# schmeing/ReSeq

Hardware: AMD Instinct MI355X
Metric: simulated read-pairs/sec (2x150 bp) (higher is better)
Workload: dtype f64

## Files before the change

reseq_amd/csrc/rsq_host.cpp:

```cpp
#include <stdio.h>
#include "rsq_host.h"
#include "rsq_textio.h"

#include <errno.h>
#include <fcntl.h>
#include <string.h>
#include <sys/mman.h>
#include <sys/stat.h>
#include <unistd.h>
#include <zlib.h>

#include <algorithm>
#include <array>
#include <atomic>
#include <chrono>
#include <exception>
#include <memory>
#include <mutex>

#include <fstream>
#include <thread>

#include "rsq_core.h"

namespace rsq {

Options &options() {
    static Options o;
    return o;
}
namespace {
struct OptionEntry {
    const char *name;
    int64_t Options::*field;
};
const OptionEntry kOptionTable[] = {
    {"fill_mode", &Options::fill_mode},         {"image_tiles", &Options::image_tiles},     {"rate_rows", &Options::rate_rows},
    {"no_indel_skip", &Options::no_indel_skip}, {"force_exact", &Options::force_exact},     {"min_quality_quads", &Options::min_quality_quads},
    {"trace_plan", &Options::trace_plan},       {"trace_prepare", &Options::trace_prepare},
    {"bias_window", &Options::bias_window},     {"window_chunks", &Options::window_chunks}, {"serial_fasta", &Options::serial_fasta},   {"trace_load", &Options::trace_load},
    {"chain_chunk", &Options::chain_chunk},     {"chain_warmup", &Options::chain_warmup},
    {"serial_parse", &Options::serial_parse},   {"parse_stretch", &Options::parse_stretch}, {"mapped_parses", &Options::mapped_parses},
    {"fasta_stretch", &Options::fasta_stretch}, {"overlap", &Options::overlap}, {"specialize", &Options::specialize}, {"job_write_direct", &Options::job_write_direct},             {"job_chunk_bytes", &Options::job_chunk_bytes}, {"host_gzip", &Options::host_gzip}, {"fill_waves", &Options::fill_waves}, {"fasta_no_stage", &Options::fasta_no_stage},
    {"hiprtc_by_name", &Options::hiprtc_by_name}, {"gzip_route", &Options::gzip_route},       {"gzip_stretch", &Options::gzip_stretch},
    {"sieve_lds", &Options::sieve_lds},         {"sieve_lds_bytes", &Options::sieve_lds_bytes}, {"sieve_tracks_mb", &Options::sieve_tracks_mb},
    {"wide_rows", &Options::wide_rows},
};
}
bool set_option(const char *name, int64_t value) {
    for (const OptionEntry &e : kOptionTable)
        if (0 == strcmp(name, e.name)) {
            options().*(e.field) = value;
            return true;
        }
    return false;
}
bool get_option(const char *name, int64_t *value) {
    for (const OptionEntry &e : kOptionTable)
        if (0 == strcmp(name, e.name)) {
            *value = options().*(e.field);
            return true;
        }
    return false;
}
const char *option_names() {
    static const std::string names = [] {
        std::string s;
        for (const OptionEntry &e : kOptionTable) s += (s.empty() ? "" : " ") + std::string(e.name);
        return s;
    }();
    return names.c_str();
}

static size_t pad8(size_t n) { return (8 - (n & 7)) & 7; }

Container::Container(const std::string &path) {
    std::ifstream f(path, std::ios::binary | std::ios::ate);
    if (!f) throw Error("cannot open profile '" + path + "'");
    std::streamsize sz = f.tellg();
    f.seekg(0);
    buf_.resize((size_t)sz);
    if (!f.read(reinterpret_cast<char *>(buf_.data()), sz)) throw Error("cannot read profile '" + path + "'");
    if (buf_.size() < 16 || memcmp(buf_.data(), "RSQPROF1", 8) != 0) throw Error("'" + path + "' is not an RSQP profile container");
    uint32_t version, n;
    memcpy(&version, &buf_[8], 4);
    memcpy(&n, &buf_[12], 4);
    if (version != 1) throw Error("unsupported RSQP version");
    static const size_t kSize[7] = {1, 2, 4, 8, 4, 8, 8};
    size_t pos = 16;
    for (uint32_t i = 0; i < n; ++i) {
        if (pos + 4 > buf_.size()) throw Error("truncated RSQP container");
// ... 1212 lines not shown
```

reseq_amd/csrc/rsq_host.h:

```cpp
#pragma once
#include <stdint.h>

#include <map>
#include <stdexcept>
#include <string>
#include <string.h>
#include <vector>

namespace rsq {

struct Error : std::runtime_error {
    using std::runtime_error::runtime_error;
};

struct Options {
    int64_t fill_mode = -1;
    int64_t image_tiles = 0;
    int64_t rate_rows = 0;
    int64_t no_indel_skip = 0;
    int64_t force_exact = 0;
    int64_t min_quality_quads = 0;
    int64_t trace_plan = 0;
    int64_t trace_prepare = 0;
    int64_t bias_window = 0;
    int64_t window_chunks = 0;
    int64_t trace_load = 0;
    int64_t serial_fasta = 0;
    int64_t fasta_stretch = 0;
    int64_t chain_chunk = 0;
    int64_t chain_warmup = -1;
    int64_t serial_parse = 0;
    int64_t mapped_parses = 0;
    int64_t parse_stretch = 0;
    int64_t job_chunk_bytes = 0;
    int64_t job_write_direct = 0;
    int64_t specialize = 1;
    int64_t fasta_no_stage = 0;
    int64_t fill_waves = 0;
    int64_t host_gzip = 0;
    int64_t gzip_route = -1;
    int64_t gzip_stretch = 0;
    int64_t hiprtc_by_name = 0;
    int64_t sieve_lds = 1;
    int64_t sieve_lds_bytes = 0;
    int64_t sieve_tracks_mb = 4096;
    int64_t wide_rows = 0;
    int64_t overlap = 0;
};
Options &options();
bool set_option(const char *name, int64_t value);
bool get_option(const char *name, int64_t *value);
const char *option_names();

struct Array {
    int dtype = 0;
    std::vector<uint64_t> dims;
    uint64_t count = 0;
    const uint8_t *data = nullptr;
};

class Container {
   public:
    explicit Container(const std::string &path);
    const Array &get(const std::string &name) const;
    bool has(const std::string &name) const { return arrays_.count(name) != 0; }
    template <class T>
    std::vector<T> vec(const std::string &name, int dtype) const {
        const Array &a = get(name);
        if (a.dtype != dtype) throw Error("profile array '" + name + "' has the wrong type");
        const T *p = reinterpret_cast<const T *>(a.data);
        return std::vector<T>(p, p + a.count);
    }
// ... 161 lines not shown
```

reseq_amd/csrc/rsq_pack.h:

```cpp
#pragma once
#include <math.h>
#include <stdio.h>
#include <stdlib.h>
#include <string.h>
#include <errno.h>
#include <fcntl.h>
#include <unistd.h>

#include <algorithm>
#include <string>
#include <vector>

#include <atomic>
#include <exception>
#include <mutex>
#include <thread>

#include "rsq_host.h"
#include "rsq_chains.h"
#include "rsq_sieve.h"
#include "rsq_reads.h"

namespace rsq {

// ... 26 lines not shown

struct SimState {
    Options opt = options();
    Profile prof;
    bool has_ref = false;
    std::vector<std::string> ref_first_names, ref_ids;
    std::vector<uint32_t> seq_len;
    std::vector<uint64_t> seq_word_off, seq_base_off;
    uint64_t total_ref_size = 0;
    uint32_t chain_chunk = 256;
    std::vector<uint64_t> ref_words_host;
    uint32_t ref_code(uint32_t seq, uint32_t pos) const { return (uint32_t)(ref_words_host[seq_word_off[seq] + (pos >> 5)] >> ((pos & 31u) * 2u)) & 3u; }
    bool has_variants = false;
    uint32_t num_alleles = 1;
    int variants_mode = 0;
    std::vector<DevVariant> variants;
    std::vector<uint32_t> var_ptr;
    std::vector<uint8_t> var_bases;
    std::vector<uint16_t> var_err_fwd, var_err_rev;
    uint16_t *dev_var_err_fwd = nullptr, *dev_var_err_rev = nullptr;
    double expected_passing = 0.0;
    std::vector<AlleleVar> allele_map;
    std::vector<uint32_t> allele_map_ptr;
    std::vector<ExtraStart> extra;
    std::vector<uint32_t> extra_seq_ptr;
    std::vector<double> host_pool;
    std::vector<uint8_t> host_par0;
    std::vector<DevTable> host_dom_error, host_error_rate;
    DevSim dev{};
    NameTable names{};
    uint16_t *sys_fwd = nullptr, *sys_rev = nullptr, *adapter_sys[2] = {nullptr, nullptr};
    uint32_t rmax = 0, read_stride = 0, ops_stride = 0, max_adapter = 0, template_words = 0;
    uint64_t insert_lengths_from = 0;
    bool prepared = false;
    uint32_t prepared_lo = 0, prepared_hi = 0;
    uint64_t seed = 0, total_pairs = 0, adapter_only_pairs = 0;
    uint32_t n_groups = 0, passes = 0, total_blocks = 0;
    std::vector<uint32_t> coverage_groups, first_block, n_blocks, block_seq;
    std::vector<double> thresholds, norm_by_len, ref_seq_bias;
    std::string ref_bias_file;
    double bias_normalization = 0;
    std::string plan_note;
    int variants_mode_packed = 0;
    bool has_methylation = false;
    std::vector<uint32_t> meth_ptr_host, meth_first_host, meth_second_host;
    std::vector<double> meth_rate_host;
};

static inline uint32_t cdiv(uint64_t a, uint64_t b) { return (uint32_t)((a + b - 1) / b); }

constexpr uint32_t kLdsBudgetBytes = 160u * 1024u;
constexpr uint32_t kLdsRateRowsFirst = 64;

inline void pack_tables(SimState &s, Uploader &up) {
    const Profile &p = s.prof;
    std::vector<double> pool;
    std::vector<uint8_t> par0;
    auto pack = [&](const std::vector<HostTable> &tabs) {
        std::vector<DevTable> out(tabs.size());
        for (size_t i = 0; i < tabs.size(); ++i) {
            const HostTable &t = tabs[i];
            DevTable d{};
            d.k = (uint32_t)t.par0.size();
            for (uint32_t v : t.par0) d.max_value = std::max(d.max_value, v);
            const uint32_t kp = row_stride(d.k);
            for (uint32_t n = 0; n < t.nm; ++n) {
                d.from[n] = t.from[n];
                d.rows[n] = t.to[n] - t.from[n];
                const size_t rows = d.k ? d.rows[n] : 0;
                if (pool.size() + rows * kp > 0xFFFFFFF0ull) throw Error("probability tables exceed 2^32 entries");
                d.off[n] = (uint32_t)pool.size();
                for (size_t r = 0; r < rows; ++r) {
                    pool.insert(pool.end(), t.dim2[n].begin() + r * d.k, t.dim2[n].begin() + (r + 1) * d.k);
                    pool.insert(pool.end(), kp - d.k, 0.0);
                }
            }
            out[i] = d;
        }
        return out;
    };
    std::vector<DevTable> quality = pack(p.quality), seq_quality = pack(p.seq_quality), base_call = pack(p.base_call), dom_error = pack(p.dom_error),
                          error_rate = pack(p.error_rate), indels = pack(p.indels);

    const uint32_t T = p.n_tiles();
    LdsPlan plan{};
    auto put_par0 = [&](DevTable &d, const HostTable &t) {
        d.par0_off = (uint32_t)par0.size();
        for (uint32_t v : t.par0) par0.push_back((uint8_t)v);
    };
    auto pad_par0 = [&] { par0.resize((par0.size() + 3u) & ~(size_t)3u, 0); };
    for (size_t i = 0; i < indels.size(); ++i) put_par0(indels[i], p.indels[i]);
    pad_par0();
    const uint32_t par0_indel_bytes = (uint32_t)par0.size();
    std::vector<uint32_t> par0_tile_first(2 * T + 1, 0);
    for (uint32_t g = 0; g < 2 * T; ++g) {
        par0_tile_first[g] = (uint32_t)par0.size();
        for (uint32_t i = 0; i < 4; ++i) put_par0(quality[g * 4 + i], p.quality[g * 4 + i]);
        put_par0(seq_quality[g], p.seq_quality[g]);
        for (uint32_t i = 0; i < 20; ++i) put_par0(base_call[g * 20 + i], p.base_call[g * 20 + i]);
        pad_par0();
    }
    par0_tile_first[2 * T] = (uint32_t)par0.size();
    for (size_t i = 0; i < dom_error.size(); ++i) put_par0(dom_error[i], p.dom_error[i]);
    for (size_t i = 0; i < error_rate.size(); ++i) put_par0(error_rate[i], p.error_rate[i]);

    std::vector<float> pool32;
// ... 81 lines not shown
                g.from[n] = any ? std::min(g.from[n], d.from[n]) : d.from[n];
                to[n] = any ? std::max(to[n], d.from[n] + d.rows[n]) : d.from[n] + d.rows[n];
            }
            any = true;
        }
        for (uint32_t n = 0; n < 4; ++n) {
            const uint32_t rows = n < nm ? std::max(1u, to[n] - g.from[n]) : 0u;
            g.before[n] = g.table_rows;
            g.last[n] = rows ? rows - 1u : 0u;
            g.table_rows += rows;
        }
        g.off32 = (uint32_t)pool32.size();
        g.lds = g.lds2 = kNoLds;
        if ((pool32.size() + (uint64_t)tabs.size() * g.table_rows * slot) * sizeof(float) > 0xFFFFFFF0ull)
            throw Error("single-precision probability tables exceed 4 GB (the kernels address them by 32-bit byte offsets)");
        for (DevTable &d : tabs) {
            d.off32 = 0;
            d.f32_ok = 1;
            const uint32_t kp = row_stride(d.k);
            for (uint32_t n = 0; n < nm && d.k; ++n)
                for (uint32_t r = 0; r < d.rows[n]; ++r)
                    for (uint32_t c = 0; c < d.k; ++c) {
                        const double v = pool[d.off[n] + (size_t)r * kp + c];
                        if (!(v == 0.0 || (v >= 0x1p-60 && v <= 0x1p29))) d.f32_ok = 0;
                    }
            const bool zeros = !d.k || !d.f32_ok;
            for (uint32_t n = 0; n < nm; ++n)
                for (uint32_t r = 0; r <= g.last[n]; ++r) {
                    const int64_t own = (int64_t)g.from[n] + r - (int64_t)d.from[n];
                    const double *row = zeros ? nullptr : pool.data() + d.off[n] + (size_t)std::min<int64_t>(std::max<int64_t>(own, 0), (int64_t)d.rows[n] - 1) * kp;
                    for (uint32_t c = 0; c < slot; ++c) pool32.push_back(row && c < d.k ? (float)row[c] : 0.f);
                }
        }
        return g;
    };
    auto family_values = [&](FamilyGeo &g, const std::vector<DevTable> &tabs, uint32_t slot) {
        g.values_src = (uint32_t)par0.size();
        for (const DevTable &d : tabs)
            for (uint32_t c = 0; c < slot; ++c) par0.push_back(c < d.k ? par0[d.par0_off + c] : (uint8_t)0);
    };
    const Options &opt = s.opt;
    const uint32_t min_quads = opt.min_quality_quads > 0 ? (uint32_t)opt.min_quality_quads : 0u;
    for (uint32_t q : kQualityQuads)
        if (!plan.quads_q && q >= min_quads && quads_of(kmax_of(quality)) <= q) plan.quads_q = q;
    const bool screenable = plan.quads_q && quads_of(kmax_of(base_call)) <= kQuadsSmall && quads_of(kmax_of(indels)) <= kQuadsSmall;
    plan.slot_q = row_slot32(plan.quads_q);
    plan.slot_b = plan.slot_i = kSlotSmall;
    if (screenable) {
        plan.q = family(quality, 4, plan.slot_q);
        plan.b = family(base_call, 4, plan.slot_b);
        plan.i = family(indels, 3, plan.slot_i);
        if (!opt.no_indel_skip)
            for (DevTable &d : indels) certain_no_indel(d);
    }
    s.dev.chain_quads = 0;
    s.dev.force_exact = opt.force_exact ? 1u : 0u;
    for (uint32_t q : kChainQuads)
        if (!s.dev.chain_quads && quads_of(kmax_of(error_rate)) <= q && quads_of(kmax_of(dom_error)) <= kQuadsSmall) s.dev.chain_quads = q;
    std::vector<uint32_t> chain_sure(1, 0u);
    if (s.dev.chain_quads) {
        copy32(dom_error, 4u * kQuadsSmall);
        copy32(error_rate, 4u * s.dev.chain_quads);
        if (!opt.no_indel_skip)
            for (DevTable &d : error_rate) {
                d.sure_range = 0;
                if (!d.k || !d.f32_ok || !d.rows[0] || !d.rows[1] || !d.rows[2]) continue;
                uint32_t z = d.k;
                for (uint32_t c = 0; c < d.k; ++c)
                    if (0 == par0[d.par0_off + c]) z = c;
                if (z == d.k) continue;
                const uint32_t kp = row_stride(d.k);
                std::vector<double> worst1(d.k, 0.0);
                for (uint32_t c = 0; c < d.k; ++c)
                    for (uint32_t r = 0; r < d.rows[1] && worst1[c] >= 0.0; ++r) {
                        const double *row = pool.data() + d.off[1] + (size_t)r * kp;
                        if (row[z] > 0.0) worst1[c] = std::max(worst1[c], row[c] / row[z]);
                        else if (row[c] > 0.0) worst1[c] = -1.0;
                    }
                d.sure_range = (uint32_t)chain_sure.size();
                for (uint32_t r0 = 0; r0 < d.rows[0]; ++r0)
                    for (uint32_t r2 = 0; r2 < d.rows[2]; ++r2) {
                        const double *m0 = pool.data() + d.off[0] + (size_t)r0 * kp, *m2 = pool.data() + d.off[2] + (size_t)r2 * kp;
                        double below = 0.0, above = 0.0;
                        bool bound = m0[z] > 0.0 && m2[z] > 0.0;
                        for (uint32_t c = 0; c < d.k && bound; ++c) {
                            if (c == z) continue;
                            if (worst1[c] < 0.0) bound = false;
                            else (c < z ? below : above) += (m0[c] / m0[z]) * worst1[c] * (m2[c] / m2[z]);
                        }
                        uint32_t range = 0;
                        if (bound) {
                            const double lo = above / (1.0 + above) * (1.0 + 1e-9), hi = 1.0 / (1.0 + below) * (1.0 - 1e-9);
                            const uint32_t lo16 = (uint32_t)std::ceil(lo * 65536.0), hi16 = (uint32_t)std::floor(hi * 65536.0);
                            if (lo16 < hi16) range = lo16 | (hi16 << 16);
                        }
                        chain_sure.push_back(range);
                    }
            }
    }
    s.dev.chain_sure = up.put(chain_sure);
    if (screenable) {
        pad_par0();
        family_values(plan.q, quality, plan.slot_q);
        family_values(plan.b, base_call, plan.slot_b);
        family_values(plan.i, indels, plan.slot_i);
    }

    uint32_t rate_rows_q = ~0u, rate_rows_b = ~0u;
    if (opt.rate_rows > 0) rate_rows_q = rate_rows_b = (uint32_t)std::min<int64_t>(opt.rate_rows, 1 << 20);
    rate_rows_q = std::min(rate_rows_q, plan.q.last[3] + 1u);
    rate_rows_b = std::min(rate_rows_b, plan.b.last[3] + 1u);
    const uint64_t budget = kLdsBudgetBytes / 4u - kSchedWords;
    auto plan_image = [&](uint32_t Ti) {
        const uint32_t n_img = 2 * T / Ti;
        uint32_t par0_bytes = 0;
        for (uint32_t g = 0; g < n_img; ++g) par0_bytes = std::max(par0_bytes, par0_indel_bytes + par0_tile_first[(g + 1) * Ti] - par0_tile_first[g * Ti]);
        const uint32_t par0_words = (par0_bytes + 15u) / 16u * 4u;
        const uint32_t desc_words = (lds_desc_count(Ti) * kDescWords + 3u) / 4u * 4u + par0_words;
        const uint32_t values_words = (4 * Ti * plan.slot_q + 20 * Ti * plan.slot_b + 12 * plan.slot_i + 15u) / 16u * 4u;
        const uint32_t rows_q = plan.q.last[0] + 1 + plan.q.last[1] + 1, rows_b = plan.b.last[0] + 1, rows_b2 = plan.b.last[2] + 1, rows_i = plan.i.last[0] + 1;
        auto odd_stride = [](uint64_t floats) { return (uint32_t)(((floats / 4u) | 1u) * 4u); };
        const uint32_t stride_q = odd_stride((uint64_t)rows_q * plan.slot_q), stride_b = odd_stride((uint64_t)rows_b * plan.slot_b), stride_b2 = odd_stride((uint64_t)rows_b2 * plan.slot_b),
                       stride_i = odd_stride((uint64_t)rows_i * plan.slot_i);
        const uint64_t need_q = (uint64_t)4 * Ti * stride_q, need_b = (uint64_t)20 * Ti * stride_b, need_b2 = (uint64_t)20 * Ti * stride_b2, need_i0 = (uint64_t)12 * stride_i;
        uint64_t need = (uint64_t)desc_words + values_words + need_q + need_b;
        auto need_rate = [&](uint32_t rows_q, uint32_t rows_b) {
            return (uint64_t)4 * Ti * odd_stride((uint64_t)rows_q * plan.slot_q) + (uint64_t)20 * Ti * odd_stride((uint64_t)rows_b * plan.slot_b);
        };
        const uint32_t ring_stride = 4 * Ti * plan.slot_q;
        need += (uint64_t)kFillWavesMax * kRingRows * ring_stride;
        if (need + need_rate(1, 1) > budget) return false;
        uint32_t rq = 1, rb = 1;
        while (rq < std::min(rate_rows_q, kLdsRateRowsFirst) && need + need_rate(rq + 1, 1) <= budget) ++rq;
        const bool stage_b2 = need + need_b2 + need_rate(rq, 1) <= budget;
        if (stage_b2) need += need_b2;
        const bool stage_i0 = need + need_i0 + need_rate(rq, 1) <= budget;
        if (stage_i0) need += need_i0;
        while (rb < std::min(rate_rows_b, kLdsRateRowsFirst) && need + need_rate(rq, rb + 1) <= budget) ++rb;
        while (rq < rate_rows_q && need + need_rate(rq + 1, rb) <= budget) ++rq;
        while (rb < rate_rows_b && need + need_rate(rq, rb + 1) <= budget) ++rb;
        plan.img_tiles = Ti;
        plan.binned = (Ti < T || opt.image_tiles == 1) ? 1u : 0u;
        plan.par0_words = par0_words;
        plan.par0_indel_bytes = par0_indel_bytes;
        plan.desc_words = desc_words;
        plan.ring_stride = ring_stride;
        plan.rate_rows_q = rq;
        plan.rate_rows_b = rb;
        plan.q.values = desc_words * 4u;
        plan.b.values = plan.q.values + 4 * Ti * plan.slot_q;
        plan.i.values = plan.b.values + 20 * Ti * plan.slot_b;
        uint32_t at = desc_words + values_words;
        plan.q.lds = at, plan.q.lds_rows = rows_q, plan.q.lds_stride = stride_q, at += (uint32_t)need_q;
        plan.b.lds = at, plan.b.lds_rows = rows_b, plan.b.lds_stride = stride_b, at += (uint32_t)need_b;
        plan.b.lds2 = stage_b2 ? at : kNoLds;
        plan.b.lds2_stride = stride_b2;
        if (stage_b2) at += (uint32_t)need_b2;
        plan.i.lds = stage_i0 ? at : kNoLds;
        plan.i.lds_rows = rows_i;
        plan.i.lds_stride = stride_i;
        if (stage_i0) at += (uint32_t)need_i0;
        plan.ring_off = at;
        plan.q3_off = plan.ring_off + kFillWavesMax * kRingRows * plan.ring_stride;
        plan.q3_stride = odd_stride((uint64_t)plan.rate_rows_q * plan.slot_q);
        plan.b3_stride = odd_stride((uint64_t)plan.rate_rows_b * plan.slot_b);
        plan.b3_off = plan.q3_off + 4 * Ti * plan.q3_stride;
        plan.total_words = plan.b3_off + 20 * Ti * plan.b3_stride;
        plan.mask = plan.quads_q;
        return true;
    };
    plan.img_tiles = T;
    if (screenable && opt.fill_mode != 0) {
        const bool per_tile_first = opt.image_tiles == 1 && T > 1;
        if (!(per_tile_first && plan_image(1)) && !plan_image(T) && !(T > 1 && plan_image(1)))
            s.plan_note = "the read kernels' table image does not fit the " + std::to_string(kLdsBudgetBytes / 1024u) +
                          " KiB of local memory even for one tile: every per-base draw runs in double precision from device memory (several times slower)";
    } else if (!screenable && opt.fill_mode != 0)
        s.plan_note = "the profile's tables are outside what the screened single-precision draws are built for (more than " + std::to_string(4u * kQualityQuads[4]) +
                      " quality values, or more than 8 base-call / indel outcomes): every per-base draw runs in double precision from device memory (several times slower)";
    if ((plan.desc_words | plan.q3_off | plan.b3_off | plan.ring_off | plan.ring_stride | plan.slot_q | plan.slot_b | plan.slot_i | plan.q.off32 | plan.b.off32 | plan.i.off32 |
         (plan.mask ? plan.q.lds | plan.b.lds | (plan.b.lds2 != kNoLds ? plan.b.lds2 : 0u) | (plan.i.lds != kNoLds ? plan.i.lds : 0u) : 0u)) & 3u)
        throw Error("internal: LDS rows must start on 16-byte boundaries");
    if (opt.trace_plan)
        fprintf(stderr, "[rsq] LDS image: mask %u, %u of %u tiles per image, %u words (%u KiB), desc %u, quality slot %u, rate rows %u / %u, q3 %u b3 %u, ring %u x %u, b2 %d i0 %d\n", plan.mask,
                plan.img_tiles, T, plan.total_words, plan.total_words / 256, plan.desc_words, plan.slot_q, plan.rate_rows_q, plan.rate_rows_b, plan.q3_off, plan.b3_off, plan.ring_off,
                plan.ring_stride, (int)(plan.b.lds2 != kNoLds), (int)(plan.i.lds != kNoLds));
    s.dev.lds = plan;
    s.dev.quality = up.put(quality);
    s.dev.seq_quality = up.put(seq_quality);
    s.dev.base_call = up.put(base_call);
    s.dev.dom_error = up.put(dom_error);
    s.dev.error_rate = up.put(error_rate);
    s.dev.indels = up.put(indels);
    par0.resize(((par0.size() + 3u) & ~(size_t)3u) + (size_t)plan.par0_words * 4u + 16u, 0);
    pool.push_back(0.0);
    pool.push_back(0.0);
    pool32.resize(pool32.size() + 8, 0.f);
    s.dev.pool = up.put(pool);
    s.dev.pool32 = up.put(pool32);
    s.dev.par0 = up.put(par0);
    s.host_pool = pool;
    s.host_par0 = par0;
    s.host_dom_error = dom_error;
    s.host_error_rate = error_rate;
}

inline uint32_t effective_fill_mask(uint32_t plan_mask, int forced) { return forced == 0 ? 0u : plan_mask; }

inline void pack_profile(SimState &s, Uploader &up) {
    const Profile &p = s.prof;
    DevSim &d = s.dev;
    d.n_tiles = p.n_tiles();
    d.phred_offset = p.phred_offset;
    d.max_len_deletion = p.max_len_deletion;
    d.reset_distance = p.reset_distance;
    d.tile_cp = up.put(discrete_cp(p.tile_abundance.data(), p.tile_abundance.size()));
    d.tiles = up.put(p.tiles);
    s.rmax = 0;
    uint32_t max_adapter = 0;
    for (int seg = 0; seg < 2; ++seg) {
        const HostAdapters &a = p.adapters[seg];
        DevAdapters &da = d.adapters[seg];
        da.n = a.n();
        da.seqs = up.put(a.seqs);
        da.seq_ptr = up.put(a.seq_ptr);
        da.adapter_cp = up.put(discrete_cp(a.significant.data(), a.significant.size()));
        std::vector<double> cut_cp;
        for (uint32_t i = 0; i < a.n(); ++i) {
            std::vector<double> cp = discrete_cp(a.cut.data() + a.cut_ptr[i], a.cut_ptr[i + 1] - a.cut_ptr[i]);
            cp.resize(a.cut_ptr[i + 1] - a.cut_ptr[i]);
            cut_cp.insert(cut_cp.end(), cp.begin(), cp.end());
            max_adapter = std::max(max_adapter, a.seq_ptr[i + 1] - a.seq_ptr[i]);
        }
        cut_cp.push_back(1.0);
        da.cut_cp = up.put(cut_cp);
        da.cut_ptr = up.put(a.cut_ptr);
        da.cut_from = up.put(a.cut_from);
        s.adapter_sys[seg] = up.put(std::vector<uint16_t>(a.seqs.size() + 1, 0));
        da.sys = s.adapter_sys[seg];
// ... 1259 lines not shown
```

reseq_amd/csrc/rsq_reads.h:

```cpp
#pragma once
#include "rsq_core.h"
#include "rsq_variants.h"
#include "rsq_text.h"

namespace rsq {

struct ReadOut {
    WordColumn seq, qual, ops;
    uint32_t cur_word, cur_index;
    uint32_t seq_word, qual_word, n_put;
    RSQ_HD void put(uint32_t pos, uint32_t base, uint32_t qual_char) {
        const uint32_t sh = (pos & 3u) * 8u;
        seq_word |= base << sh;
        qual_word |= qual_char << sh;
        n_put = pos + 1u;
        if ((pos & 3u) == 3u) {
            seq.at(pos >> 2) = seq_word;
            qual.at(pos >> 2) = qual_word;
            seq_word = qual_word = 0;
        }
    }
    RSQ_HD void op(uint32_t it, uint32_t code) {
        const uint32_t wi = it >> 4;
        if (wi != cur_index) {
// ... 342 lines not shown
    RSQ_HD uint32_t org_len() const { return 0; }
    RSQ_HD uint32_t base(uint32_t) const { return 0; }
    RSQ_HD uint32_t sys_base(uint32_t) const { return 0; }
    RSQ_HD uint32_t sys_deleted(uint32_t) const { return 0; }
};

RSQ_HD uint32_t draw_tile(const DevSim &S, uint32_t c0, uint32_t c1, uint32_t c2, uint32_t c3base) {
    if (RSQ_SIM(S, n_tiles) > 1) return discrete_draw(S.tile_cp, RSQ_SIM(S, n_tiles), u32_to_unit(philox(S.seed, c0, c1, c2, c3base).w0));
    return 0;
}

RSQ_HD uint32_t lds_desc_count(uint32_t n_tiles) { return 25u * n_tiles + 12u; }
RSQ_HD uint32_t image_qbase(const DevSim &S, uint32_t seg, uint32_t first_tile) { return (seg * RSQ_SIM(S, n_tiles) + first_tile) * 4u; }
constexpr uint32_t kDescWords = sizeof(DevTable) / 4u;

#if defined(__HIP_DEVICE_COMPILE__)
#define RSQ_NOINLINE __device__ __noinline__
#else
#define RSQ_NOINLINE inline
#endif
#if defined(RSQ_SCREEN_STATS) && !defined(__HIP_DEVICE_COMPILE__)
#define RSQ_SCREEN_COUNT(family, decided) (++RSQ_SCREEN_STATS[family][0], RSQ_SCREEN_STATS[family][1] += !(decided))
#else
#define RSQ_SCREEN_COUNT(family, decided) ((void)0)
#endif

template <int NM>
#if defined(__HIP_DEVICE_COMPILE__)
__device__ __noinline__
#else
inline
#endif
    uint32_t exact_draw_call(const double *pool, const RSQ_LDS float *img, uint32_t par0_words, uint32_t desc, uint32_t i0, uint32_t i1, uint32_t i2, uint32_t i3, uint32_t word) {
    const DevTable t = reinterpret_cast<const RSQ_LDS DevTable *>(img)[desc];
    uint32_t idx[NM];
    idx[0] = i0;
    idx[1] = i1;
    idx[2] = i2;
    if constexpr (NM == 4) idx[3] = i3;
    double ps;
    const uint32_t value = draw_slim<NM>(t, pool, reinterpret_cast<const RSQ_LDS uint8_t *>(img + par0_words), idx, u32_to_unit(word), ps);
    return value | (0.0 == ps ? 0x80000000u : 0u);
}

#define RSQ_GEO_ROW(S, fam, n, v) ((uint32_t)geo_clamp((int32_t)(v) - (int32_t)RSQ_PLAN(S, fam.from[n]), (int32_t)RSQ_PLAN(S, fam.last[n])))
RSQ_HD int32_t geo_clamp(int32_t d, int32_t last) {
#if defined(__clang__)
    return __builtin_elementwise_min(__builtin_elementwise_max(d, 0), last);
#else
    return d < 0 ? 0 : (d > last ? last : d);
#endif
}

template <uint32_t MASK, int QB = RSQ_SCREEN_BATCH>
struct ScreenTables {
    using Sum = uint32_t;
    static constexpr int QQ = (int)MASK;
    const DevSim &S;
    const RSQ_LDS float *img;
    uint32_t qbase;
    const RSQ_LDS float *ring_;
    uint32_t t;
    uint32_t demand = 0xFFFFFFFFu;
    RSQ_HD DevTable desc(uint32_t local) const { return reinterpret_cast<const RSQ_LDS DevTable *>(img)[local]; }
    RSQ_HD uint32_t par0_at() const { return RSQ_PLAN(S, desc_words) - RSQ_PLAN(S, par0_words); }
    RSQ_HD DevTable quality(uint32_t i) const { return desc(i - qbase); }
    RSQ_HD DevTable seq_quality(uint32_t i) const { return desc(24u * RSQ_PLAN(S, img_tiles) + 12u + i - qbase / 4u); }
    RSQ_HD const RSQ_LDS float *ring(uint32_t p) const { return ring_ + (p % kRingSlots) * RSQ_PLAN(S, ring_stride); }
    RSQ_HD bool in_ring(uint32_t p) const { return t - p <= kRingLag; }
    template <int NM>
    RSQ_HD uint32_t exact(uint32_t desc, const uint32_t (&idx)[NM], uint32_t word, uint32_t &ps) const {
        const uint32_t r = exact_draw_call<NM>(S.pool, img, par0_at(), desc, idx[0], idx[1], idx[2], NM == 4 ? idx[NM - 1] : 0u, word);
        ps = (r >> 31) ^ 1u;
        return r & 0x7FFFFFFFu;
    }
    template <int NM>
    RSQ_HD uint32_t settle(bool decided, uint32_t values, uint32_t column, uint32_t desc, const uint32_t (&idx)[NM], uint32_t u, uint32_t &ps) const {
        uint32_t value = reinterpret_cast<const RSQ_LDS uint8_t *>(img)[values + column];
        ps = 1u;
        decided = decided && !RSQ_SIM(S, force_exact);
        if (!decided) value = exact<NM>(desc, idx, u, ps);
        return value;
    }

    RSQ_HD uint32_t draw_quality(uint32_t i, const uint32_t (&idx)[4], uint32_t u, uint32_t &ps) const {
        const uint32_t local = i - qbase, slot = RSQ_PLAN(S, slot_q), nr = RSQ_PLAN(S, rate_rows_q), r3 = RSQ_GEO_ROW(S, q, 3, idx[3]);
        const RSQ_LDS float *mine = img + RSQ_PLAN(S, q.lds) + local * RSQ_PLAN(S, q.lds_stride);
        const LdsRow32 m0{mine + RSQ_GEO_ROW(S, q, 0, idx[0]) * slot}, m1{mine + (RSQ_PLAN(S, q.before[1]) + RSQ_GEO_ROW(S, q, 1, idx[1])) * slot};
        const bool near = in_ring(idx[2]);
        const LdsRow32 m2{ring_ + (near ? idx[2] % kRingSlots : kRingSlots) * RSQ_PLAN(S, ring_stride) + local * slot};
        const LdsRow32 m3{img + RSQ_PLAN(S, q3_off) + local * RSQ_PLAN(S, q3_stride) + (r3 < nr ? r3 : 0u) * slot};
        uint32_t col = 0;
        const bool decided = draw_screened_batched<QQ, QQ % QB == 0 ? QB : (QQ % 2 == 0 ? 2 : 1)>(u, col, m0, m1, m2, m3) && (near || idx[2] == demand) && r3 < nr;
        RSQ_SCREEN_COUNT(0, decided);
        return settle<4>(decided, RSQ_PLAN(S, q.values), local * slot + col, local, idx, u, ps);
    }
    RSQ_HD uint32_t draw_base_call(uint32_t i, const uint32_t (&idx)[4], uint32_t u, uint32_t &ps) const {
        const uint32_t local = i - qbase * 5u, slot = RSQ_PLAN(S, slot_b), nr = RSQ_PLAN(S, rate_rows_b), r3 = RSQ_GEO_ROW(S, b, 3, idx[3]);
        const uint32_t g = 4u * (RSQ_PLAN(S, b.off32) + i * (RSQ_PLAN(S, b.table_rows) * slot));
        const LdsRow32 m0{img + RSQ_PLAN(S, b.lds) + local * RSQ_PLAN(S, b.lds_stride) + RSQ_GEO_ROW(S, b, 0, idx[0]) * slot};
        const PoolRow32 m1{S.pool32, g + 4u * (RSQ_PLAN(S, b.before[1]) + RSQ_GEO_ROW(S, b, 1, idx[1])) * slot};
        const uint32_t r2 = RSQ_GEO_ROW(S, b, 2, idx[2]);
        const bool m2_staged = RSQ_PLAN(S, b.lds2) != kNoLds, staged = r3 < nr;
        const MixedRow32 m2{LdsRow32{img + (m2_staged ? RSQ_PLAN(S, b.lds2) + local * RSQ_PLAN(S, b.lds2_stride) + r2 * slot : 0u)},
                            PoolRow32{S.pool32, g + 4u * (RSQ_PLAN(S, b.before[2]) + r2) * slot}, m2_staged};
        const MixedRow32 m3{LdsRow32{img + RSQ_PLAN(S, b3_off) + local * RSQ_PLAN(S, b3_stride) + (staged ? r3 : 0u) * slot}, PoolRow32{S.pool32, g + 4u * (RSQ_PLAN(S, b.before[3]) + r3) * slot}, staged};
        uint32_t col = 0;
        const bool decided = draw_screened<(int)kQuadsSmall>(u, col, m0, m1, m2, m3);
        RSQ_SCREEN_COUNT(1, decided);
        return settle<4>(decided, RSQ_PLAN(S, b.values), local * slot + col, 4u * RSQ_PLAN(S, img_tiles) + local, idx, u, ps);
    }
    RSQ_HD uint32_t draw_indel(uint32_t i, const uint32_t (&idx)[3], uint32_t u, uint32_t &ps) const {
        const RSQ_LDS DevTable *d = reinterpret_cast<const RSQ_LDS DevTable *>(img) + (24u * RSQ_PLAN(S, img_tiles) + i);
        const uint32_t range = d->sure_range, lo16 = range & 0xFFFFu;
        const bool sure = (u >> 16) - lo16 < (range >> 16) - lo16 && idx[0] <= d->from[0];
        RSQ_SCREEN_COUNT(3, sure);
        ps = 1u;
        if (sure) return 0;
        const uint32_t slot = RSQ_PLAN(S, slot_i), r0 = RSQ_GEO_ROW(S, i, 0, idx[0]);
        const uint32_t g = 4u * (RSQ_PLAN(S, i.off32) + i * (RSQ_PLAN(S, i.table_rows) * slot));
        const bool m0_staged = RSQ_PLAN(S, i.lds) != kNoLds;
        const MixedRow32 m0{LdsRow32{img + (m0_staged ? RSQ_PLAN(S, i.lds) + i * RSQ_PLAN(S, i.lds_stride) + r0 * slot : 0u)}, PoolRow32{S.pool32, g + 4u * r0 * slot}, m0_staged};
        const PoolRow32 m1{S.pool32, g + 4u * (RSQ_PLAN(S, i.before[1]) + RSQ_GEO_ROW(S, i, 1, idx[1])) * slot}, m2{S.pool32, g + 4u * (RSQ_PLAN(S, i.before[2]) + RSQ_GEO_ROW(S, i, 2, idx[2])) * slot};
        uint32_t col = 0;
        const bool decided = draw_screened<(int)kQuadsSmall>(u, col, m0, m1, m2);
        RSQ_SCREEN_COUNT(2, decided);
        return settle<3>(decided, RSQ_PLAN(S, i.values), i * slot + col, 24u * RSQ_PLAN(S, img_tiles) + i, idx, u, ps);
    }
    RSQ_HD uint32_t draw_seq_quality(uint32_t i, const uint32_t (&idx)[3], uint32_t u, uint32_t &ps) const {
        const uint32_t r = exact_draw_call<3>(S.pool, img, par0_at(), 24u * RSQ_PLAN(S, img_tiles) + 12u + i - qbase / 4u, idx[0], idx[1], idx[2], 0u, u);
        ps = (r >> 31) ^ 1u;
        return r & 0x7FFFFFFFu;
    }
};

RSQ_HD void lds_stage_descriptors(const DevSim &S, RSQ_LDS float *img, uint32_t qbase, uint32_t tid, uint32_t nthreads) {
    const uint32_t T = RSQ_PLAN(S, img_tiles);
    RSQ_LDS uint32_t *dst = reinterpret_cast<RSQ_LDS uint32_t *>(img);
    const uint32_t wq = 4u * T * kDescWords, wb = 20u * T * kDescWords, wi = 12u * kDescWords, ws = T * kDescWords;
    const uint32_t *q = reinterpret_cast<const uint32_t *>(S.quality + qbase), *b = reinterpret_cast<const uint32_t *>(S.base_call + qbase * 5u),
                   *in = reinterpret_cast<const uint32_t *>(S.indels), *sq = reinterpret_cast<const uint32_t *>(S.seq_quality + qbase / 4u);
    const uint32_t tiles_at = S.quality[qbase].par0_off, shift = tiles_at - RSQ_PLAN(S, par0_indel_bytes);
    for (uint32_t i = tid; i < wq; i += nthreads) dst[i] = q[i] - (i % kDescWords == 1u ? shift : 0u);
    for (uint32_t i = tid; i < wb; i += nthreads) dst[wq + i] = b[i] - (i % kDescWords == 1u ? shift : 0u);
    for (uint32_t i = tid; i < wi; i += nthreads) dst[wq + wb + i] = in[i];
    for (uint32_t i = tid; i < ws; i += nthreads) dst[wq + wb + wi + i] = sq[i] - (i % kDescWords == 1u ? shift : 0u);
    const uint32_t *p0 = reinterpret_cast<const uint32_t *>(S.par0), *p1 = reinterpret_cast<const uint32_t *>(S.par0 + tiles_at);
    const uint32_t indel_words = RSQ_PLAN(S, par0_indel_bytes) / 4u, par0_at = RSQ_PLAN(S, desc_words) - RSQ_PLAN(S, par0_words);
    for (uint32_t i = tid; i < RSQ_PLAN(S, par0_words); i += nthreads) dst[par0_at + i] = i < indel_words ? p0[i] : p1[i - indel_words];
    const uint32_t nq = T * RSQ_PLAN(S, slot_q), nb = 5u * T * RSQ_PLAN(S, slot_b), ni = 3u * RSQ_PLAN(S, slot_i);
    const uint32_t *vq = reinterpret_cast<const uint32_t *>(S.par0 + RSQ_PLAN(S, q.values_src)) + qbase / 4u * RSQ_PLAN(S, slot_q),
                   *vb = reinterpret_cast<const uint32_t *>(S.par0 + RSQ_PLAN(S, b.values_src)) + qbase / 4u * 5u * RSQ_PLAN(S, slot_b),
                   *vi = reinterpret_cast<const uint32_t *>(S.par0 + RSQ_PLAN(S, i.values_src));
    for (uint32_t i = tid; i < nq; i += nthreads) dst[RSQ_PLAN(S, q.values) / 4u + i] = vq[i];
    for (uint32_t i = tid; i < nb; i += nthreads) dst[RSQ_PLAN(S, b.values) / 4u + i] = vb[i];
    for (uint32_t i = tid; i < ni; i += nthreads) dst[RSQ_PLAN(S, i.values) / 4u + i] = vi[i];
}
RSQ_HD void lds_stage_family_rows(const DevSim &S, RSQ_LDS float *img, uint32_t off32, uint32_t table_rows, uint32_t first, uint32_t n_tables, uint32_t first_row, uint32_t n_rows,
                                  uint32_t slot, uint32_t dst_off, uint32_t dst_stride, uint32_t tid, uint32_t nthreads) {
    const uint32_t per_table = n_rows * (slot / 4u);
    for (uint32_t i = tid; i < n_tables * per_table; i += nthreads) {
        const uint32_t table = i / per_table, g = i - table * per_table;
        reinterpret_cast<RSQ_LDS Quad *>(img + dst_off + table * dst_stride)[g] = reinterpret_cast<const Quad *>(S.pool32 + off32 + ((size_t)(first + table) * table_rows + first_row) * slot)[g];
    }
}
RSQ_HD void lds_stage_rows(const DevSim &S, RSQ_LDS float *img, uint32_t qbase, uint32_t tid, uint32_t nthreads) {
    const uint32_t T = RSQ_PLAN(S, img_tiles), sq = RSQ_PLAN(S, slot_q), sb = RSQ_PLAN(S, slot_b), si = RSQ_PLAN(S, slot_i);
    lds_stage_family_rows(S, img, RSQ_PLAN(S, q.off32), RSQ_PLAN(S, q.table_rows), qbase, 4u * T, 0u, RSQ_PLAN(S, q.lds_rows), sq, RSQ_PLAN(S, q.lds), RSQ_PLAN(S, q.lds_stride), tid, nthreads);
    lds_stage_family_rows(S, img, RSQ_PLAN(S, b.off32), RSQ_PLAN(S, b.table_rows), qbase * 5u, 20u * T, 0u, RSQ_PLAN(S, b.lds_rows), sb, RSQ_PLAN(S, b.lds), RSQ_PLAN(S, b.lds_stride), tid, nthreads);
    if (RSQ_PLAN(S, b.lds2) != kNoLds)
        lds_stage_family_rows(S, img, RSQ_PLAN(S, b.off32), RSQ_PLAN(S, b.table_rows), qbase * 5u, 20u * T, RSQ_PLAN(S, b.before[2]), RSQ_PLAN(S, b.last[2]) + 1u, sb, RSQ_PLAN(S, b.lds2),
                              RSQ_PLAN(S, b.lds2_stride), tid, nthreads);
    if (RSQ_PLAN(S, i.lds) != kNoLds)
        lds_stage_family_rows(S, img, RSQ_PLAN(S, i.off32), RSQ_PLAN(S, i.table_rows), 0u, 12u, 0u, RSQ_PLAN(S, i.lds_rows), si, RSQ_PLAN(S, i.lds), RSQ_PLAN(S, i.lds_stride), tid, nthreads);
    lds_stage_family_rows(S, img, RSQ_PLAN(S, q.off32), RSQ_PLAN(S, q.table_rows), qbase, 4u * T, RSQ_PLAN(S, q.before[3]), RSQ_PLAN(S, rate_rows_q), sq, RSQ_PLAN(S, q3_off), RSQ_PLAN(S, q3_stride), tid,
                          nthreads);
    lds_stage_family_rows(S, img, RSQ_PLAN(S, b.off32), RSQ_PLAN(S, b.table_rows), qbase * 5u, 20u * T, RSQ_PLAN(S, b.before[3]), RSQ_PLAN(S, rate_rows_b), sb, RSQ_PLAN(S, b3_off), RSQ_PLAN(S, b3_stride), tid,
                          nthreads);
}
RSQ_HD uint32_t lds_ring_items(const DevSim &S) { return 4u * RSQ_PLAN(S, img_tiles) * RSQ_PLAN(S, quads_q); }
struct RingItem {
    uint32_t rows;
    uint32_t at;
};
RSQ_HD RingItem lds_ring_item(const DevSim &S, uint32_t qbase, uint32_t item) {
    const uint32_t table = item / RSQ_PLAN(S, quads_q), c = item % RSQ_PLAN(S, quads_q), slot = RSQ_PLAN(S, slot_q);
    return RingItem{4u * (RSQ_PLAN(S, q.off32) + ((qbase + table) * RSQ_PLAN(S, q.table_rows) + RSQ_PLAN(S, q.before[2])) * slot + 4u * c), table * slot + 4u * c};
}
RSQ_HD Quad lds_ring_load(const DevSim &S, const RingItem &it, uint32_t p) { return PoolRow32{S.pool32, it.rows + 4u * RSQ_GEO_ROW(S, q, 2, p) * RSQ_PLAN(S, slot_q)}.quad(0u); }
RSQ_HD void lds_ring_store(const DevSim &S, const RingItem &it, RSQ_LDS float *ring, uint32_t p, const Quad &q) {
    *reinterpret_cast<RSQ_LDS Quad *>(ring + (p % kRingSlots) * RSQ_PLAN(S, ring_stride) + it.at) = q;
}
RSQ_HD void lds_ring_stage(const DevSim &S, const RingItem &it, RSQ_LDS float *ring, uint32_t p) { lds_ring_store(S, it, ring, p, lds_ring_load(S, it, p)); }
RSQ_HD void lds_ring_stage_demand(const DevSim &S, const RingItem &it, RSQ_LDS float *ring, uint32_t p) {
    *reinterpret_cast<RSQ_LDS Quad *>(ring + kRingSlots * RSQ_PLAN(S, ring_stride) + it.at) = lds_ring_load(S, it, p);
}
RSQ_HD void lds_ring_stage(const DevSim &S, uint32_t qbase, RSQ_LDS float *ring, uint32_t p, uint32_t item) { lds_ring_stage(S, lds_ring_item(S, qbase, item), ring, p); }
RSQ_HD FragmentSrc fragment_src(const DevSim &S, const Fragment &f, uint32_t seg, uint32_t end) {
    const uint32_t L = S.seq_len[f.seq];
    const uint32_t want = S.read_lengths[seg].to + RSQ_SIM(S, max_len_deletion);
    FragmentSrc src;
    src.words = hap_words(S, f.allele);
    src.word_off = S.seq_word_off[f.seq];
    src.len = f.len < want ? f.len : want;
    src.reverse = seg != f.strand;
    src.first = src.reverse ? end : f.start;
    src.sys_ = src.reverse ? S.sys_rev + S.seq_base_off[f.seq] + (L - end) : S.sys_fwd + S.seq_base_off[f.seq] + f.start;
    src.converted = nullptr;
    src.gc_prefix = hap_gc_prefix(S, f.allele);
    return src;
}
RSQ_HD FragmentSrc fragment_src(const DevSim &S, const Fragment &f, uint32_t seg) { return fragment_src(S, f, seg, f.start + f.len); }

struct VariantSrc : FragmentSrc {
    const DevVariant *var;
    const uint16_t *err;
    uint32_t n_var, L, allele;
    uint32_t *walk_error;
    uint32_t spos0, cur0, var_pos0;
    mutable uint32_t spos, cur, var_pos;
    RSQ_HD const DevVariant &var_at(uint32_t i) const { return reverse ? var[n_var - 1u - i] : var[i]; }
    RSQ_HD uint32_t var_spos(uint32_t i) const { return reverse ? L - 1u - var_at(i).pos : var_at(i).pos; }
    RSQ_HD uint32_t var_err(uint32_t i, uint32_t k) const { return err[var_at(i).off + k]; }
    RSQ_HD uint32_t lower_bound(uint32_t sp) const {
        uint32_t lo = 0, hi = n_var;
        while (lo < hi) {
            const uint32_t mid = (lo + hi) >> 1;
            if (var_spos(mid) < sp) lo = mid + 1u;
            else hi = mid;
        }
        return lo;
// ... 592 lines not shown
```

reseq_amd/csrc/rsq_types.h:

```cpp
#pragma once
#if defined(__HIPCC_RTC__)
using __hip_internal::int32_t;
using __hip_internal::int64_t;
using __hip_internal::uint16_t;
using __hip_internal::uint32_t;
using __hip_internal::uint64_t;
using __hip_internal::uint8_t;
typedef unsigned long uintptr_t;
#define RSQ_DEVICE_BUILD 1
#define RSQ_HD __host__ __device__ __forceinline__
#elif defined(__HIPCC__)
#include <stdint.h>
#include <hip/hip_runtime.h>
#define RSQ_DEVICE_BUILD 1
#define RSQ_HD __host__ __device__ __forceinline__
#else
#include <stdint.h>
#define RSQ_DEVICE_BUILD 0
#define RSQ_HD inline
#endif

namespace rsq {

constexpr uint32_t kBlockSize = 1000;
// ... 20 lines not shown
static_assert(__builtin_offsetof(DevTable, par0_off) == 4, "lds_stage_descriptors rewrites word 1 of a descriptor");
constexpr uint32_t kNoLds = 0xFFFFFFFFu;
#ifndef RSQ_CHUNK_LARGE
#define RSQ_CHUNK_LARGE 4
#endif
constexpr uint32_t kChunkSmall = 3, kChunkLarge = RSQ_CHUNK_LARGE;
RSQ_HD uint32_t chunk_pairs(uint32_t k) { return k <= 2u * kChunkSmall ? kChunkSmall : kChunkLarge; }
RSQ_HD uint32_t chunks_of(uint32_t k, uint32_t u) { return (k + 2u * u - 1u) / (2u * u); }
RSQ_HD uint32_t row_stride(uint32_t k) {
    const uint32_t u = chunk_pairs(k), kp = chunks_of(k, u) * 2u * u;
    return (kp & 2u) ? kp : kp + 2u;
}
RSQ_HD uint32_t quads_of(uint32_t k) { return (k + 3u) / 4u; }
RSQ_HD uint32_t row_slot32(uint32_t quads) {
    const uint32_t w = quads * 4u;
    return (w & 4u) ? w : w + 4u;
}
constexpr uint32_t kQuadsSmall = 2, kSlotSmall = 8;
constexpr uint32_t kQualityQuads[] = {3, 6, 10, 11, 12};
constexpr uint32_t kChainQuads[] = {8, 16, 26};
constexpr uint32_t kRingSlots = 2, kRingLag = 1;
constexpr uint32_t kRingRows = kRingSlots + 1u;

struct FamilyGeo {
    uint32_t from[4];
    uint32_t last[4];
    uint32_t before[4];
    uint32_t table_rows;
    uint32_t off32;
    uint32_t lds;
    uint32_t lds_rows;
    uint32_t lds_stride;
    uint32_t lds2;
    uint32_t lds2_stride;
    uint32_t values;
    uint32_t values_src;
};

struct LdsPlan {
    uint32_t mask;
    uint32_t img_tiles;
    uint32_t binned;
    uint32_t desc_words;
    uint32_t par0_words;
    uint32_t par0_indel_bytes;
    uint32_t slot_q, slot_b, slot_i;
    uint32_t quads_q;
    uint32_t rate_rows_q, rate_rows_b;
    uint32_t q3_off, b3_off;
    uint32_t q3_stride, b3_stride;
    uint32_t ring_off, ring_stride;
    uint32_t total_words;
    FamilyGeo q, b, i;
};

struct Fragment {
    uint32_t seq;
    uint32_t start;
    uint32_t len;
    uint16_t dup;
    uint8_t strand;
    uint8_t allele;
    uint32_t block;
    uint32_t number;
};

struct ReadMeta {
    uint16_t read_len;
    uint16_t num_errors;
    uint16_t n_iter_m;
    uint16_t n_iter_s;
    uint16_t hard_clip;
    uint16_t tile_id;
    uint16_t cigar_chars;
    uint16_t plain;
};

struct DevVariant {
    uint32_t pos;
    uint32_t len;
    uint32_t off;
    uint32_t pad;
    uint64_t allele[2];
};
struct AlleleVar {
    uint32_t pos;
    uint32_t vid;
    int32_t shift;
    int32_t gc;
};
struct FragmentVar {
    uint32_t end;
    uint32_t sub;
    int32_t start_var;
    uint32_t start_var_pos;
    int32_t end_var;
    uint32_t end_var_pos;
};
struct ExtraStart {
    uint32_t pos;
    uint32_t sub;
    int32_t first_variant_id;
    uint32_t start_variant_pos;
};

struct DevAdapters {
    uint32_t n;
// ... 105 lines not shown
```

Baseline: 248.3 million.

## Add LDS-staged word screen to skip exact base-call draws

On the host, compute per-table conservative float bounds on the ratio of non-reference to reference base-call probabilities, bucketed over the four conditioning indices. These bounds are packed into pool32 and staged into LDS when the budget allows. In the kernel, the draw first checks whether the uniform word is certain to land on the reference base. If so, it returns that base directly and skips the four-row table lookup and cumulative comparison. The cost is extra LDS space, which can reduce rate rows staged elsewhere, plus a short check on every draw.

```diff
diff --git a/reseq_amd/csrc/rsq_host.cpp b/reseq_amd/csrc/rsq_host.cpp
--- a/reseq_amd/csrc/rsq_host.cpp
+++ b/reseq_amd/csrc/rsq_host.cpp
@@ -36,7 +36,7 @@
 };
 const OptionEntry kOptionTable[] = {
     {"fill_mode", &Options::fill_mode},         {"image_tiles", &Options::image_tiles},     {"rate_rows", &Options::rate_rows},
-    {"no_indel_skip", &Options::no_indel_skip}, {"force_exact", &Options::force_exact},     {"min_quality_quads", &Options::min_quality_quads},
+    {"no_indel_skip", &Options::no_indel_skip}, {"force_exact", &Options::force_exact},     {"base_call_word", &Options::base_call_word},     {"min_quality_quads", &Options::min_quality_quads},
     {"trace_plan", &Options::trace_plan},       {"trace_prepare", &Options::trace_prepare},
     {"bias_window", &Options::bias_window},     {"window_chunks", &Options::window_chunks}, {"serial_fasta", &Options::serial_fasta},   {"trace_load", &Options::trace_load},
     {"chain_chunk", &Options::chain_chunk},     {"chain_warmup", &Options::chain_warmup},
diff --git a/reseq_amd/csrc/rsq_host.h b/reseq_amd/csrc/rsq_host.h
--- a/reseq_amd/csrc/rsq_host.h
+++ b/reseq_amd/csrc/rsq_host.h
@@ -18,6 +18,7 @@
     int64_t image_tiles = 0;
     int64_t rate_rows = 0;
     int64_t no_indel_skip = 0;
+    int64_t base_call_word = 1;
     int64_t force_exact = 0;
     int64_t min_quality_quads = 0;
     int64_t trace_plan = 0;
diff --git a/reseq_amd/csrc/rsq_pack.h b/reseq_amd/csrc/rsq_pack.h
--- a/reseq_amd/csrc/rsq_pack.h
+++ b/reseq_amd/csrc/rsq_pack.h
@@ -102,6 +102,65 @@
 constexpr uint32_t kLdsBudgetBytes = 160u * 1024u;
 constexpr uint32_t kLdsRateRowsFirst = 64;
 
+struct WordScreenGeo {
+    uint32_t at[4], cap[4], stride;
+};
+inline WordScreenGeo word_screen_geo(const FamilyGeo &g) {
+    WordScreenGeo w{};
+    const uint32_t lim[4] = {kWordCapQuality, kWordCapBuckets, kWordCapErrors, kWordCapRate};
+    uint32_t at = 0;
+    for (uint32_t n = 0; n < 4; ++n) {
+        const uint32_t top = (g.from[n] + g.last[n]) >> (1 == n ? kWordPosShift : 0u);
+        w.at[n] = at;
+        w.cap[n] = std::min(top, lim[n]);
+        at += w.cap[n] + 1u;
+    }
+    w.stride = at;
+    return w;
+}
+inline bool base_call_word_bounds(const DevTable &d, const double *pool, const uint8_t *par0, uint32_t base, const FamilyGeo &g, const WordScreenGeo &w, float *out, uint32_t *sides) {
+    const float inf = __builtin_inff();
+    std::fill(out, out + 2u * w.stride, inf);
+    if (!d.k || d.k > 8u || !d.f32_ok || !d.rows[0] || !d.rows[1] || !d.rows[2] || !d.rows[3]) return false;
+    uint32_t z = d.k;
+    for (uint32_t c = d.k; c--;)
+        if (par0[d.par0_off + c] == base) z = c;
+    if (z == d.k) return false;
+    const uint32_t kp = row_stride(d.k);
+    auto stored = [&](double x) {
+        if (!(x > 0.0)) return 0.f;
+        if (x > 0x1p100) return inf;
+        x *= 1.0 + 0x1p-21;
+        float f = (float)x;
+        if ((double)f < x) f = nextafterf(f, inf);
+        return f < 0x1p-30f ? 0x1p-30f : f;
+    };
+    for (uint32_t n = 0; n < 4; ++n)
+        for (uint32_t e = 0; e <= w.cap[n]; ++e) {
+            const uint32_t sh = 1 == n ? kWordPosShift : 0u, lo_v = e << sh, hi_v = e < w.cap[n] ? ((e + 1u) << sh) - 1u : std::max(lo_v, g.from[n] + g.last[n]);
+            double side[2] = {0.0, 0.0};
+            for (uint32_t v = lo_v; v <= hi_v; ++v) {
+                const int64_t own = (int64_t)v - (int64_t)d.from[n];
+                const double *row = pool + d.off[n] + (size_t)std::min<int64_t>(std::max<int64_t>(own, 0), (int64_t)d.rows[n] - 1) * kp;
+                double got[2] = {0.0, 0.0};
+                for (uint32_t c = 0; c < d.k; ++c) {
+                    if (c == z) continue;
+                    double &x = got[c > z];
+                    if (row[z] > 0.0) x = 0 == n ? x + row[c] / row[z] : std::max(x, row[c] / row[z]);
+                    else if (row[c] > 0.0) x = (double)inf;
+                }
+                side[0] = std::max(side[0], got[0]);
+                side[1] = std::max(side[1], got[1]);
+            }
+            float *o = out + 2u * (w.at[n] + e);
+            o[0] = stored(side[0]);
+            o[1] = stored(side[1]);
+        }
+    for (uint32_t n = 0; n < 4; ++n)
+        for (uint32_t e = 0; e <= w.cap[n]; ++e) *sides |= (out[2u * (w.at[n] + e)] > 0.f ? 1u : 0u) | (out[2u * (w.at[n] + e) + 1u] > 0.f ? 2u : 0u);
+    return true;
+}
+
 inline void pack_tables(SimState &s, Uploader &up) {
     const Profile &p = s.prof;
     std::vector<double> pool;
@@ -289,6 +348,25 @@
         plan.i = family(indels, 3, plan.slot_i);
         if (!opt.no_indel_skip)
             for (DevTable &d : indels) certain_no_indel(d);
+    }
+    plan.bw_off = kNoLds;
+    const bool word_screen = screenable && opt.base_call_word != 0;
+    const WordScreenGeo wg = word_screen_geo(plan.b);
+    if (word_screen) {
+        std::vector<float> pairs(base_call.size() * 2u * wg.stride);
+        uint32_t sides = 0;
+        for (size_t i = 0; i < base_call.size(); ++i)
+            base_call_word_bounds(base_call[i], pool.data(), par0.data(), (uint32_t)(i / 5u % 4u), plan.b, wg, pairs.data() + i * 2u * wg.stride, &sides);
+        if (!sides) sides = 1u;
+        const uint32_t width = 3u == sides ? 2u : 1u;
+        plan.bw_sides = sides;
+        plan.bw_stride = (wg.stride * width + 3u) & ~3u;
+        plan.bw_src = (uint32_t)pool32.size();
+        pool32.resize(pool32.size() + base_call.size() * plan.bw_stride, 0.f);
+        for (size_t i = 0; i < base_call.size(); ++i)
+            for (uint32_t e = 0; e < wg.stride; ++e)
+                for (uint32_t h = 0; h < width; ++h) pool32[plan.bw_src + i * plan.bw_stride + e * width + h] = pairs[(i * wg.stride + e) * 2u + (2u == width ? h : sides - 1u)];
+        for (uint32_t n = 0; n < 4; ++n) plan.bw_at[n] = wg.at[n], plan.bw_cap[n] = wg.cap[n];
     }
     s.dev.chain_quads = 0;
     s.dev.force_exact = opt.force_exact ? 1u : 0u;
@@ -367,6 +445,9 @@
         const uint32_t ring_stride = 4 * Ti * plan.slot_q;
         need += (uint64_t)kFillWavesMax * kRingRows * ring_stride;
         if (need + need_rate(1, 1) > budget) return false;
+        const uint64_t need_bw = (uint64_t)20 * Ti * plan.bw_stride;
+        const bool stage_bw = word_screen && need + need_bw + need_rate(1, 1) <= budget;
+        if (stage_bw) need += need_bw;
         uint32_t rq = 1, rb = 1;
         while (rq < std::min(rate_rows_q, kLdsRateRowsFirst) && need + need_rate(rq + 1, 1) <= budget) ++rq;
         const bool stage_b2 = need + need_b2 + need_rate(rq, 1) <= budget;
@@ -402,7 +483,8 @@
         plan.q3_stride = odd_stride((uint64_t)plan.rate_rows_q * plan.slot_q);
         plan.b3_stride = odd_stride((uint64_t)plan.rate_rows_b * plan.slot_b);
         plan.b3_off = plan.q3_off + 4 * Ti * plan.q3_stride;
-        plan.total_words = plan.b3_off + 20 * Ti * plan.b3_stride;
+        plan.bw_off = stage_bw ? plan.b3_off + 20 * Ti * plan.b3_stride : kNoLds;
+        plan.total_words = plan.b3_off + 20 * Ti * plan.b3_stride + (stage_bw ? (uint32_t)need_bw : 0u);
         plan.mask = plan.quads_q;
         return true;
     };
@@ -418,10 +500,13 @@
     if ((plan.desc_words | plan.q3_off | plan.b3_off | plan.ring_off | plan.ring_stride | plan.slot_q | plan.slot_b | plan.slot_i | plan.q.off32 | plan.b.off32 | plan.i.off32 |
          (plan.mask ? plan.q.lds | plan.b.lds | (plan.b.lds2 != kNoLds ? plan.b.lds2 : 0u) | (plan.i.lds != kNoLds ? plan.i.lds : 0u) : 0u)) & 3u)
         throw Error("internal: LDS rows must start on 16-byte boundaries");
-    if (opt.trace_plan)
+    if (opt.trace_plan) {
         fprintf(stderr, "[rsq] LDS image: mask %u, %u of %u tiles per image, %u words (%u KiB), desc %u, quality slot %u, rate rows %u / %u, q3 %u b3 %u, ring %u x %u, b2 %d i0 %d\n", plan.mask,
                 plan.img_tiles, T, plan.total_words, plan.total_words / 256, plan.desc_words, plan.slot_q, plan.rate_rows_q, plan.rate_rows_b, plan.q3_off, plan.b3_off, plan.ring_off,
                 plan.ring_stride, (int)(plan.b.lds2 != kNoLds), (int)(plan.i.lds != kNoLds));
+        fprintf(stderr, "[rsq] word screen of the base call: %s, %u words per table (caps %u %u %u %u), %s\n", plan.bw_off != kNoLds ? "staged" : "none", plan.bw_stride, plan.bw_cap[0],
+                plan.bw_cap[1], plan.bw_cap[2], plan.bw_cap[3], 3u == plan.bw_sides ? "both ends" : (2u == plan.bw_sides ? "lower end only" : "upper end only"));
+    }
     s.dev.lds = plan;
     s.dev.quality = up.put(quality);
     s.dev.seq_quality = up.put(seq_quality);
diff --git a/reseq_amd/csrc/rsq_reads.h b/reseq_amd/csrc/rsq_reads.h
--- a/reseq_amd/csrc/rsq_reads.h
+++ b/reseq_amd/csrc/rsq_reads.h
@@ -418,6 +418,24 @@
 #endif
 }
 
+#if defined(RSQ_WORD_SCREEN_STATS) && !defined(__HIP_DEVICE_COMPILE__)
+#define RSQ_WORD_SCREEN_COUNT(sure) RSQ_WORD_SCREEN_STATS(sure)
+#else
+#define RSQ_WORD_SCREEN_COUNT(sure) ((void)0)
+#endif
+
+RSQ_HD bool word_screen_sure(const Float2 &a, const Float2 &p, const Float2 &e, const Float2 &r, uint32_t word, uint32_t sides) {
+    const Float2 f = ((a * p) * e) * r;
+    const float uf = (float)word * 2.3283064365386963e-10f;
+    bool sure = true;
+    if (sides & 1u) sure = fma1(uf, f.x, uf) < 0.99999904632568359375f;
+    if (sides & 2u) {
+        const float om = 1.f - uf;
+        sure = sure && f.y < 512.f && fma1(om, f.y, om) < 0.9998779296875f;
+    }
+    return sure;
+}
+
 template <uint32_t MASK, int QB = RSQ_SCREEN_BATCH>
 struct ScreenTables {
     using Sum = uint32_t;
@@ -461,8 +479,33 @@
         RSQ_SCREEN_COUNT(0, decided);
         return settle<4>(decided, RSQ_PLAN(S, q.values), local * slot + col, local, idx, u, ps);
     }
+    RSQ_HD bool base_call_word(uint32_t local, const uint32_t (&idx)[4], uint32_t u) const {
+        if (RSQ_PLAN(S, bw_off) == kNoLds || RSQ_SIM(S, force_exact)) return false;
+        const RSQ_LDS float *mine = img + RSQ_PLAN(S, bw_off) + local * RSQ_PLAN(S, bw_stride);
+        const uint32_t sides = RSQ_PLAN(S, bw_sides);
+        auto entry = [&](uint32_t n, uint32_t value) {
+            const uint32_t e = RSQ_PLAN(S, bw_at[n]) + (value < RSQ_PLAN(S, bw_cap[n]) ? value : RSQ_PLAN(S, bw_cap[n]));
+            Float2 f;
+            if (3u == sides) f = *reinterpret_cast<const RSQ_LDS Float2 *>(mine + 2u * e);
+            else {
+                const float x = mine[e];
+                f.x = 2u == sides ? 0.f : x;
+                f.y = 2u == sides ? x : 0.f;
+            }
+            return f;
+        };
+        return word_screen_sure(entry(0, idx[0]), entry(1, idx[1] >> kWordPosShift), entry(2, idx[2]), entry(3, idx[3]), u, sides);
+    }
     RSQ_HD uint32_t draw_base_call(uint32_t i, const uint32_t (&idx)[4], uint32_t u, uint32_t &ps) const {
-        const uint32_t local = i - qbase * 5u, slot = RSQ_PLAN(S, slot_b), nr = RSQ_PLAN(S, rate_rows_b), r3 = RSQ_GEO_ROW(S, b, 3, idx[3]);
+        const uint32_t local = i - qbase * 5u;
+        const bool sure = base_call_word(local, idx, u);
+        RSQ_WORD_SCREEN_COUNT(sure);
+        if (sure) {
+            RSQ_SCREEN_COUNT(1, true);
+            ps = 1u;
+            return ((local * 52429u) >> 18) & 3u;
+        }
+        const uint32_t slot = RSQ_PLAN(S, slot_b), nr = RSQ_PLAN(S, rate_rows_b), r3 = RSQ_GEO_ROW(S, b, 3, idx[3]);
         const uint32_t g = 4u * (RSQ_PLAN(S, b.off32) + i * (RSQ_PLAN(S, b.table_rows) * slot));
         const LdsRow32 m0{img + RSQ_PLAN(S, b.lds) + local * RSQ_PLAN(S, b.lds_stride) + RSQ_GEO_ROW(S, b, 0, idx[0]) * slot};
         const PoolRow32 m1{S.pool32, g + 4u * (RSQ_PLAN(S, b.before[1]) + RSQ_GEO_ROW(S, b, 1, idx[1])) * slot};
@@ -543,6 +586,10 @@
                           nthreads);
     lds_stage_family_rows(S, img, RSQ_PLAN(S, b.off32), RSQ_PLAN(S, b.table_rows), qbase * 5u, 20u * T, RSQ_PLAN(S, b.before[3]), RSQ_PLAN(S, rate_rows_b), sb, RSQ_PLAN(S, b3_off), RSQ_PLAN(S, b3_stride), tid,
                           nthreads);
+    if (RSQ_PLAN(S, bw_off) != kNoLds) {
+        const float *src = S.pool32 + RSQ_PLAN(S, bw_src) + (size_t)qbase * 5u * RSQ_PLAN(S, bw_stride);
+        for (uint32_t i = tid; i < 20u * T * RSQ_PLAN(S, bw_stride); i += nthreads) img[RSQ_PLAN(S, bw_off) + i] = src[i];
+    }
 }
 RSQ_HD uint32_t lds_ring_items(const DevSim &S) { return 4u * RSQ_PLAN(S, img_tiles) * RSQ_PLAN(S, quads_q); }
 struct RingItem {
diff --git a/reseq_amd/csrc/rsq_types.h b/reseq_amd/csrc/rsq_types.h
--- a/reseq_amd/csrc/rsq_types.h
+++ b/reseq_amd/csrc/rsq_types.h
@@ -96,7 +96,12 @@
     uint32_t ring_off, ring_stride;
     uint32_t total_words;
     FamilyGeo q, b, i;
-};
+    uint32_t bw_off, bw_stride;
+    uint32_t bw_src;
+    uint32_t bw_at[4], bw_cap[4];
+    uint32_t bw_sides;
+};
+constexpr uint32_t kWordPosShift = 4, kWordCapQuality = 95, kWordCapBuckets = 63, kWordCapErrors = 3, kWordCapRate = 63;
 
 struct Fragment {
     uint32_t seq;
```

Measured after the change: 265.7 million (median of 6 runs). 1.07x the previous value.
